# tomer196/GaUDI

Measured on AMD Instinct MI355X. Metric: guided molecules/sec (1000-step), higher is better.
Workload: dtype f32

## Files before the change

gaudi_amd/csrc/sampler_kernel.h:

```cpp
#pragma once
#include "edm_device.h"
#include "pred_device.h"
#include "w8_edm.h"
#include "w8_pred.h"

#ifndef GAUDI_STATIC_PRIO
#define GAUDI_STATIC_PRIO 0
#endif

namespace gaudi {

enum Mode { MODE_PHI = 0, MODE_SAMPLE = 1, MODE_PRED_FWD = 2, MODE_PRED_GRAD = 3, MODE_GUIDE = 4, MODE_NLL = 5 };

struct KParams {
  int mode, B, N, F, EW;
  int NR;
  int do_init, do_decode, guided;
  int s_hi, s_lo, T;
  const float* node_mask;
  const int* order;
  const uint32_t* edges;
  const float* emask;
  const int* npairs;
  const uint32_t* seginfo;
// ... 289 lines not shown
    base += align16((N + 1 + S + 1) / 2);
    for (int i = tid; i < N; i += kThreads) sSeg[i] = P.seginfo[b * N + i];
    for (int i = tid; i < N + 1; i += kThreads) sOff[i] = P.soff[(size_t)b * (N + 1) + i];
    for (int i = tid; i < S; i += kThreads) {
      sEdge[i] = P.edges[(size_t)b * S + i];
      sEm[i] = P.emask[(size_t)b * S + i];
      sIdx[i] = P.sidx[(size_t)b * S + i];
    }
    mg.N = N; mg.D = 3 + P.F; mg.S = S;
    mg.NC = P.ncols[b];
    mg.ntiles = P.npairs[b];
    mg.rounds = (mg.ntiles + w8::kWaves - 1) / w8::kWaves;
    mg.pubx = P.pubx;
    mg.pub_ch = P.pub_ch;
    mg.hk = P.hk_off;
    mg.side = P.side_off;
    mg.mask = sMask; mg.edge = sEdge; mg.em = sEm; mg.seg = sSeg; mg.soff = sOff; mg.sidx = sIdx;
    return base;
  }
  __device__ __forceinline__ static void set_rows(Graph& mg, const int* row, int ncomp, int NR) { mg.row = row; mg.ncomp = ncomp; mg.NR = NR; }
  __device__ __forceinline__ static Graph8Args gargs(const Graph& mg) {
    return Graph8Args{mg.N, mg.D, mg.S, mg.NC, mg.ntiles, mg.pubx, mg.pub_ch, mg.hk};
  }
  static constexpr bool kGlobalNodes = GN != 0 || PG;
  template <int HP>
  __device__ __forceinline__ static void edm(const EdmDev& W, const Graph& mg, float* net, const float* sZ, float* sEps,
                                             float* sMean, float t_val, int tid STAMP_DECL, float* gnode) {
#ifdef GAUDI_STAMPS
    w8::NetSmem<HP, SP, GN> sm;
    sm.carve(net, mg.N, mg.S, GN ? uni(gnode) : nullptr);
    sm.hk = w8::lds_at(mg.hk);
    w8::edm_forward<HP, SP, GN>(W, mg, sm, sZ, sEps, sMean, t_val, tid STAMP_ARGS);
#else
    (void)net; (void)sZ; (void)sEps; (void)sMean; (void)tid;
    edm8_call<HP, SP, GN, kFL>(W, gargs(mg), t_val, gnode);
#endif
  }
  template <int HP>
  __device__ __forceinline__ static void guide(const PredDev& W, const Graph& mg, float* net, float* sZ, float* sGrad, float* sTmp,
                                               float* sMean, float t_val, float sigma, const float* target_w, float scale,
                                               float* pred_out, float readout_div, float* stash, int tid STAMP_DECL, int phase,
                                               const float* dpred_ext, float* gnode, const float* dz_ext, const VtDev* vt,
                                               int b, int srow) {
#ifdef GAUDI_STAMPS
    (void)vt; (void)b; (void)srow;
    (void)dz_ext;
    w8::guidance_update<HP, SP, MR, GN, PG>(W, mg, net, sZ, sGrad, sTmp, sMean, t_val, sigma, target_w, scale, pred_out, readout_div, stash,
                                            mg.pubx, mg.pub_ch, tid STAMP_ARGS, phase, dpred_ext, (GN || PG) ? uni(gnode) : nullptr);
#else
    (void)sTmp;
    w8::PredSmem<HP, SP, GN, PG> sm;
    sm.carve(net, mg.N, mg.S, mg.pubx, gnode);
    if (phase != 2) pred_fwd8_call<HP, SP, MR, GN, kFL, PG, SD>(W, gargs(mg), t_val, stash, readout_div, gnode, SD != 0 ? mg.side : 0);
    if (vt != nullptr) vt_seed8(vt, b, srow, W.K, (int)(sm.pred - lds_base()));
    else w8::guidance_seed(W, sm, target_w, scale, pred_out, tid, phase, dpred_ext);
    if (phase == 1) return;
    pred_bwd8_call<HP, SP, MR, GN, kFL, PG>(W, gargs(mg), stash, readout_div, phase == 2 ? 1 : 0, gnode);
    if (dz_ext != nullptr) {
      for (int e = tid; e < mg.N * mg.D; e += kThreads) sGrad[e] += dz_ext[e];
      __syncthreads();
    }
    if (vt != nullptr) vt_norm8(vt, b, srow, W.K, mg.N * mg.D, (int)(sGrad - lds_base()));
    w8::guidance_apply(mg, sZ, sGrad, sMean, sigma, tid);
    if (vt != nullptr) vt_clip8(vt, b, srow, W.K, (int)(sMean - lds_base()));
#endif
  }
  template <int HP>
  __device__ __forceinline__ static void pred_entry(const PredDev& W, const Graph& mg, float* net, float* sZ, float* sGrad,
                                                    float* sTmp, float* sMean, float t_val, const float* dpred, bool want_grad,
                                                    float* pred_out, float readout_div, float* stash, int tid STAMP_DECL, float* gnode) {
    w8::predictor_entry<HP, SP, MR, GN, PG>(W, mg, net, sZ, sGrad, sTmp, sMean, t_val, dpred, want_grad, pred_out, readout_div, stash, mg.pubx,
                            mg.pub_ch, tid STAMP_ARGS, gnode);
  }
};
using V8 = V8T<0>;
using V8S = V8T<1>;
using V8H = V8T<2>;

__host__ __device__ inline int common_floats_base(int N, int D) { return 3 * align16(N * D) + align16(N) + 16; }

// ... 361 lines not shown
```

gaudi_amd/csrc/w8_edm.h:

```cpp
#pragma once
#include "edm_device.h"
#include "w8_common.h"
#include "w8_split.h"
#include "w8_nodes_f16.h"

namespace gaudi {
namespace w8 {

__host__ __device__ constexpr int gn_lds_buffers(int gn) { return gn == 2 ? 2 : 0; }
template <int HP, int SP = 0, int GN = 0>
struct NetSmem {
  static constexpr bool kGlobalNodes = GN != 0;
  float *h, *p, *q;
  float *agg, *agg1;
  float* ring;
  float *x, *x0;
  uint32_t *pmax, *qmax;
  float* hsc;
  f4* geo;
  float* d0;
  float* trans;
  float* vec;
  float* hk = nullptr;
  __host__ __device__ static int floats(int N, int S) {
// ... 115 lines not shown
    const float* ew = w + lay.emb_w();
    const float* eb = w + lay.emb_b();
    for (int idx = tid; idx < N * HP; idx += kThreads) {
      const int n = idx / HP, f = idx % HP;
      float acc = 0.f;
      const float m = mg.mask[n];
      for (int k = 0; k < F; ++k) acc += gload(ew + f * F1 + k) * (sZ[n * D + 3 + k] * m);
      acc += gload(ew + f * F1 + F) * t_val;
      sm.h[n * LD + f] = acc + gload(eb + f);
    }
  }
  __syncthreads();
  compute_geo(sm, mg, 0.f, tid, true);
  typename EdgeRing<HP, SP>::type ring;
  er_init<HP>(ring, sm.ring, W.ktail != 0, W.ws, W.hinv);
  static_assert(SP == 0 || NodeMath<SP>::kF16, "the split edge GEMMs take their column scales from the fp16 node GEMMs' row maxima");
  constexpr bool NH = NodeMath<SP>::kF16;
  constexpr bool RI = node_ring_idle(HP, SP, GN);
  constexpr bool STG = GN && !NH;
  float* const xs0 = sm.ring;
  float* const xs1 = sm.ring + stage_stride(N * LD);
  if constexpr (!RI) er_start<HP>(ring, wbe, lay.gcl(0, 0) + 2 * PK, wave, lane);
  typename NodePFSel<HP, NH>::type pf;
  node_prefetch_x<HP, NH, kAheadOne>(pf, wb, wbe, lay.gcl(0, 0), mg.NC, wave, lane, tw);
  auto hctx = [&]() {
    if constexpr (NH) {
      if constexpr (RI) return node_ctx_h<HP>(sm.ring, EdgeRing<HP, SP>::kFloats, mg.NC, W.hinv, tw, sm.hsc);
      else return node_ctx_h<HP>(ring.slot(ring.par ^ 1), EdgeRing<HP, SP>::kFloats / 2, mg.NC, W.hinv, tw, sm.hsc);
    } else {
      return NodeCtxH{1.f, nullptr, nullptr, tw, nullptr};
    }
  };
  const bool keep = NH && sm.hk != nullptr;
  bool h_kept = false;
  constexpr int NV = (7 * HP + 16 + kThreads - 1) / kThreads;
  VecPF<NV> vpf;
  vec_prefetch<NV, kThreads>(vpf, wb, lay.gcl(0, 0) + 6 * PK, 7 * HP + 16, tid);
  STAMP(ST_EDM_IO);

  for (int l = 0; l < W.L; ++l) {
    compute_geo(sm, mg, W.norm_constant, tid, false);
    STAMP(ST_GEO);
    for (int s = 0; s < W.S; ++s) {
      const int G = lay.gcl(l, s);
      const int Wnext_edge = s + 1 < W.S ? lay.gcl(l, s + 1) + 2 * PK : lay.equ(l) + 2 * PK;
      if constexpr (STG) stage_rows(xs0, sm.h, N * LD, wave, lane);
      for (int idx = tid; idx < N * (LD / 4); idx += kThreads) {
// ... 209 lines not shown
```

gaudi_amd/csrc/w8_nodes_f16.h:

```cpp
#pragma once
#include "w8_split.h"

namespace gaudi {
namespace w8 {


constexpr float kLoScale = 2048.f;
#ifndef GAUDI_NODE_ABLATE
#define GAUDI_NODE_ABLATE 0
#endif
constexpr int kAblateH = GAUDI_NODE_ABLATE;
#ifndef GAUDI_NODE_STAMPS
#define GAUDI_NODE_STAMPS 0
#endif
#ifndef GAUDI_NODE_PRIO
#define GAUDI_NODE_PRIO 1
#endif
struct NodeStampH {
  unsigned long long sum[8], last;
  __device__ __forceinline__ void start() { last = __builtin_amdgcn_s_memtime(); }
  __device__ __forceinline__ void mark(int i) {
    const unsigned long long t = __builtin_amdgcn_s_memtime();
    sum[i] += t - last;
    last = t;
// ... 103 lines not shown
}
template <int HP, class SRC>
__device__ __forceinline__ void split_rows_h(const SplitBufH& sb, const SRC& X_, int N, int wave, int lane) {
  const auto X = rows_of(X_);
  for (int n = wave; n < N; n += 2 * kWaves) {
    const int n2 = n + kWaves < N ? n + kWaves : n;
    SplitRowH a = split_row_load<HP>(X, n, lane), b = split_row_load<HP>(X, n2, lane);
    a.mx = wave_max_u32(a.mx);
    b.mx = wave_max_u32(b.mx);
    split_row_store<HP>(sb, a.x, a.mx, n, lane);
    if (n2 != n) split_row_store<HP>(sb, b.x, b.mx, n2, lane);
  }
}

__device__ __forceinline__ void lds_barrier() {
  asm volatile("s_waitcnt lgkmcnt(0)" ::: "memory");
  __builtin_amdgcn_s_barrier();
  asm volatile("" ::: "memory");
}

#ifndef GAUDI_NODE_DEPTH
#define GAUDI_NODE_DEPTH 3
#endif
#ifndef GAUDI_NODE_LATE
#define GAUDI_NODE_LATE 0
#endif
#ifndef GAUDI_NODE_TAIL_EARLY
#define GAUDI_NODE_TAIL_EARLY 0
#endif
template <int HP>
struct NodeGeoH {
  static constexpr int T = HP / 16;
  static constexpr int NTW = T > kWaves ? 2 : 1;
  static constexpr int nc = nh_chunks(HP);
  static constexpr int D = nc < GAUDI_NODE_DEPTH ? (nc > 0 ? nc : 1) : GAUDI_NODE_DEPTH;
  static constexpr bool odd = nh_odd(HP);
};
template <int NTW>
struct NodeSetH {
  u4 p[NTW][2];
};
template <int HP>
struct NodePFH {
  NodeSetH<NodeGeoH<HP>::NTW> s[NodeGeoH<HP>::D];
};

constexpr int kOOBBytes = (int)0x80000000u;
template <int HP>
struct TileLanesH {
  int vo[NodeGeoH<HP>::NTW];
  __device__ __forceinline__ TileLanesH(int wave, int lane, bool on = true) {
#pragma unroll
    for (int u = 0; u < NodeGeoH<HP>::NTW; ++u)
      vo[u] = (on && wave + kWaves * u < NodeGeoH<HP>::T) ? lane * 16 + (wave + kWaves * u) * 2048 : kOOBBytes;
  }
};
template <int HP, int NU = NodeGeoH<HP>::NTW>
__device__ __forceinline__ void nh_load(NodeSetH<NodeGeoH<HP>::NTW>& s, const WBuf& wh, int chunk_off, const TileLanesH<HP>& tl) {
#pragma unroll
  for (int u = 0; u < NU; ++u) {
    s.p[u][0] = __builtin_bit_cast(u4, __builtin_amdgcn_raw_buffer_load_b128(wh.r, tl.vo[u], chunk_off * 4, GAUDI_NODE_LOAD_AUX));
    s.p[u][1] = __builtin_bit_cast(u4, __builtin_amdgcn_raw_buffer_load_b128(wh.r, tl.vo[u] + 1024, chunk_off * 4, GAUDI_NODE_LOAD_AUX));
  }
}
constexpr int kAheadOne = 1, kAheadAll = 99;
template <int HP, int AHEAD = kAheadAll>
__device__ __forceinline__ void node_prefetch_h(NodePFH<HP>& pf, const WBuf& wh, int W , int wave, int lane) {
  constexpr int nd = AHEAD < NodeGeoH<HP>::D ? AHEAD : NodeGeoH<HP>::D;
  const TileLanesH<HP> tl(wave, lane);
  static_for<nd>([&](auto d_tag) {
    constexpr int d = decltype(d_tag)::value;
    nh_load<HP>(pf.s[d], wh, 2 * W + d * nh_chunk_floats(HP), tl);
  });
}

constexpr int kNodePlain = 0;
constexpr int kNodeFresh = 1;
constexpr int kNodeOneTile = 2;
constexpr int kTailRuntime = 0;
constexpr int kTailOne = 1;

struct NodeCtxH {
  float winv;
  float* split_a;
  float* split_b;
  bool ktail;
  float* scales;
  float* scales_b = nullptr;
};

struct YInitBias {};
struct YInitRows {
  const float* y;
};
template <int HP, int EPI, bool TWO, int MAXNT, int PIN = kAheadOne, int POUT = kAheadOne, int FL = kNodePlain, int TAIL = kTailRuntime,
          int NU = 0, class XB = const float*, class XA = const float*, class YI = YInitBias>
__device__ __forceinline__ void node_gemm_h(const WBuf& wh, int Wa, const XA& sXa, bool do_split_a, int Wb, const XB& sXb,
                                            const float* sBias, float* sY, const float* sRes, const float* sMask, int N, int wave,
                                            int lane, const NodeCtxH& cx, NodePFH<HP>& pf, int nextW = -1, float* gPre = nullptr,
                                            uint32_t* sMaxOut = nullptr ,
                                            NodeStampH* ns = nullptr, const YI& yinit = YI{}) {
  (void)ns;
  (void)yinit;
  using G = NodeGeoH<HP>;
  constexpr int T = G::T, LD = HP + 4, NTW = NU > 0 ? NU : G::NTW, nc = G::nc, D = G::D;
  constexpr int kIn = PIN < D ? PIN : D, kOut = POUT < D ? POUT : D;
  constexpr int kLate = nc < D ? 0 : (GAUDI_NODE_LATE < kOut ? GAUDI_NODE_LATE : kOut);
  constexpr int TQ = TAIL == kTailOne ? 1 : 4;
  const bool ktail = TAIL == kTailOne ? true : cx.ktail;
  constexpr bool kFresh = FL == kNodeFresh;
  const int c = lane & 15, g = lane >> 4;
  const int nt = (MAXNT < 2 || N <= 16) ? 1 : (MAXNT < 3 || N <= 32) ? 2 : 3;
  const bool seq = TWO && cx.split_b == cx.split_a;
  const SplitBufH sa{cx.split_a, nt, cx.scales}, sb{cx.split_b, nt, cx.scales_b != nullptr ? cx.scales_b : cx.scales + kScaleFloatsH};
  const int bpos = nh_bpos(c, g);
  const TileLanesH<HP> tl(wave, lane);
  const TileLanesH<HP> tl_next(wave, lane, nextW >= 0);
  const int Wn = nextW >= 0 ? nextW : Wa;
  static_for<D>([&](auto d_tag) {
    constexpr int d = decltype(d_tag)::value;
    if constexpr (d >= kIn) nh_load<HP, NTW>(pf.s[d], wh, 2 * Wa + d * nh_chunk_floats(HP), tl);
  });
  float ta[NTW][TQ], tb[NTW][TQ];
  if constexpr (G::odd) {
#pragma unroll
    for (int u = 0; u < NTW; ++u) {
      const int t = wave + kWaves * u < T ? wave + kWaves * u : 0;
#pragma unroll
      for (int q = 0; q < TQ; ++q) {
        const int ln = ((q == 0 || !ktail) && wave + kWaves * u < T) ? lane : kOOBLane;
// ... 40 lines not shown
#pragma unroll
    for (int u = 0; u < NTW; ++u) acc1[j][u] = mfma_h(s.p[u][0], b.l, acc1[j][u]);
#pragma unroll
    for (int u = 0; u < NTW; ++u) acc0[j][u] = mfma_h(s.p[u][0], b.h, acc0[j][u]);
#pragma unroll
    for (int u = 0; u < NTW; ++u) acc1[j][u] = mfma_h(s.p[u][1], b.h, acc1[j][u]);
  };
  auto tail_steps = [&](const SplitBufH& s_, const float (&tw)[NTW][TQ], auto j_tag) {
    constexpr int j = decltype(j_tag)::value;
    if constexpr (G::odd) {
      const float* xt = s_.tail(HP) + j * 256 + g * 16 + c;
#pragma unroll
      for (int u = 0; u < NTW; ++u) y[j][u] = mfma1(tw[u][0], xt[0], y[j][u]);
      if constexpr (TQ > 1) {
        if (!ktail) {
#pragma unroll
          for (int q = 1; q < TQ; ++q)
#pragma unroll
            for (int u = 0; u < NTW; ++u) y[j][u] = mfma1(tw[u][q], xt[64 * q], y[j][u]);
        }
      }
    }
  };
  constexpr bool kTailEarly = GAUDI_NODE_TAIL_EARLY != 0;
  auto tail_early = [&](const SplitBufH& s_, const float (&tw)[NTW][TQ]) {
    if constexpr (kTailEarly && G::odd)
      static_for<MAXNT>([&](auto j_tag) {
        if (decltype(j_tag)::value < nt) tail_steps(s_, tw, j_tag);
      });
  };
  auto fold = [&](const SplitBufH& s_, const float (&tw)[NTW][TQ]) {
    static_for<MAXNT>([&](auto j_tag) {
      constexpr int j = decltype(j_tag)::value;
      if (j < nt) {
        if constexpr (!kTailEarly) tail_steps(s_, tw, j_tag);
        const float sc = s_.scale(HP)[j * 16 + c] * cx.winv;
#pragma unroll
        for (int u = 0; u < NTW; ++u) {
          y[j][u] = y[j][u] + (acc0[j][u] + acc1[j][u] * (1.0f / kLoScale)) * sc;
          acc0[j][u] = splat(0.f);
          acc1[j][u] = splat(0.f);
        }
      }
    });
  };
  auto source = [&](auto src_tag, const SplitBufH& s_) {
    constexpr int src = decltype(src_tag)::value;
    constexpr bool last_src = !TWO || src == 1;
    const int Wcur = src == 0 ? Wa : Wb;
    BH bcur = bld(s_, 0, 0);
    static_for<nc>([&](auto i_tag) {
      constexpr int i = decltype(i_tag)::value;
      constexpr int d = i % D;
      BH bnext = bcur;
      if constexpr (i + 1 < nc) bnext = bld(s_, i + 1, 0);
      __builtin_amdgcn_sched_barrier(0);
      mm(pf.s[d], bcur, 0);
      if constexpr (MAXNT >= 2) {
        if (nt >= 2) {
          mm(pf.s[d], bld(s_, i, 1), 1);
          if constexpr (MAXNT >= 3) {
            if (nt >= 3) mm(pf.s[d], bld(s_, i, 2), 2);
          }
        }
      }
      __builtin_amdgcn_sched_barrier(0);
      if (!(kAblateH & 4)) {
        if constexpr (i + D < nc) nh_load<HP, NTW>(pf.s[d], wh, 2 * Wcur + (i + D) * nh_chunk_floats(HP), tl);
        else if constexpr (!last_src) nh_load<HP, NTW>(pf.s[d], wh, 2 * Wb + d * nh_chunk_floats(HP), tl);
        else if constexpr (d < kOut - kLate) nh_load<HP, NTW>(pf.s[d], wh, 2 * Wn + d * nh_chunk_floats(HP), tl_next);
      }
      __builtin_amdgcn_sched_barrier(0);
      bcur = bnext;
    });
  };
  auto late = [&](auto d_tag) {
    constexpr int d = decltype(d_tag)::value;
    if constexpr (d >= kOut - kLate && d < kOut) {
      __builtin_amdgcn_sched_barrier(0);
      if (!(kAblateH & 4)) nh_load<HP, NTW>(pf.s[d], wh, 2 * Wn + d * nh_chunk_floats(HP), tl_next);
      __builtin_amdgcn_sched_barrier(0);
    }
  };
  NSTAMP(3);
#if GAUDI_NODE_PRIO
  if constexpr (!kFresh)
    if ((GAUDI_NODE_PRIO == 1 && wave >= kWaves / 2) || (GAUDI_NODE_PRIO == 2 && wave < kWaves / 2)) __builtin_amdgcn_s_setprio(1);
#endif
  tail_early(sa, ta);
  source(std::integral_constant<int, 0>{}, sa);
  NSTAMP(4);
  if constexpr (!TWO) late(std::integral_constant<int, kOut - kLate>{});
  fold(sa, ta);
  NSTAMP(5);
  if constexpr (TWO) {
    if (seq) {
      lds_barrier();
      split_rows_h<HP>(sb, sXb, N, wave, kFresh ? fresh(lane) : lane);
      lds_barrier();
    }
    tail_early(sb, tb);
    source(std::integral_constant<int, 1>{}, sb);
    late(std::integral_constant<int, kOut - kLate>{});
    fold(sb, tb);
  }
  static_for<D>([&](auto d_tag) {
    if constexpr (decltype(d_tag)::value > kOut - kLate) late(d_tag);
  });
#if GAUDI_NODE_PRIO
  if constexpr (!kFresh) __builtin_amdgcn_s_setprio(0);
#endif
  const int le = kFresh ? fresh(lane) : lane, ce = le & 15, ge = le >> 4;
  static_for<MAXNT>([&](auto j_tag) {
    constexpr int j = decltype(j_tag)::value;
    if (j < nt) {
#pragma unroll
      for (int u = 0; u < NTW; ++u) {
        const int t = wave + kWaves * u;
        const int nd = j * 16 + ce;
        f4 yy = y[j][u];
        if (t < T && nd < N) {
          float* dst = sY + nd * LD + 16 * t + 4 * ge;
          const bool pad = G::odd && ktail && t == T - 1 && ge > 0;
          if (pad) yy = splat(0.f);
          if (gPre != nullptr) nstash_store((f4*)(gPre + nd * HP + 16 * t + 4 * ge), yy);
          if (sMaxOut != nullptr) atomicMax(sMaxOut + nd, umax(umax(absbits(yy[0]), absbits(yy[1])), umax(absbits(yy[2]), absbits(yy[3]))));
          if (!pad) {
            if (EPI == EPI_SILU) yy = silu4v(yy);
            if (EPI == EPI_RESIDUAL_MASK) {
              const f4 r = *(const f4*)(sRes + nd * LD + 16 * t + 4 * ge);
              yy = (r + yy) * sMask[nd];
// ... 108 lines not shown
    side_compute<HP, s>(job, a, lane);
    __builtin_amdgcn_sched_barrier(0);
    side_issue<HP, s + 1>(job, a, lane);
    __builtin_amdgcn_sched_barrier(0);
    ring.par ^= 1;
  });
}

#ifndef GAUDI_NODE_F16
#define GAUDI_NODE_F16 1
#endif
template <int SP>
struct NodeMath {
  static constexpr bool kF16 = SP != 0 && GAUDI_NODE_F16 != 0;
};
template <int HP, bool NH>
struct NodePFSel {
  using type = NodePF<HP>;
};
template <int HP>
struct NodePFSel<HP, true> {
  using type = NodePFH<HP>;
};
template <int HP, bool NH, int AHEAD, class PF>
__device__ __forceinline__ void node_prefetch_x(PF& pf, const WBuf& wb, const WBuf& wbe, int W, int N, int wave, int lane, bool tw) {
  if constexpr (NH) node_prefetch_h<HP, AHEAD>(pf, wbe, W, wave, lane);
  else node_prefetch<HP>(pf, wb, W, wave, lane, tw);
}
template <int HP, int EPI, bool TWO, int GN, bool NH, int PIN, int POUT, int FL = kNodePlain, int XBS = 0, class PF>
__device__ __forceinline__ void node_gemm_x(const WBuf& wb, const WBuf& wbe, int Wa, const float* Xa, const float* XaS, bool split_a, int Wb,
                                            const float* Xb, const float* XbS, const float* sBias, float* sY, const float* sRes,
                                            const float* sMask, int N, int wave, int lane, bool tw, const NodeCtxH& cx, PF& pf,
                                            int nextW = -1, float* gPre = nullptr, uint32_t* sMaxOut = nullptr,
                                            const float* Xb1 = nullptr, float xb_div = 1.f) {
  static_assert(XBS == 0 || (NH && GN == 0 && TWO), "summed second sources: the fp16-pair form of the resident kernels");
  if constexpr (NH) {
    constexpr int MAXNT = GN ? 3 : FL == kNodeOneTile ? 1 : 2;
    constexpr int TAIL = FL == kNodeOneTile && nh_odd(HP) ? kTailOne : kTailRuntime;
    if constexpr (XBS == 0)
      node_gemm_h<HP, EPI, TWO, MAXNT, PIN, POUT, FL, TAIL>(wbe, Wa, Xa, split_a, Wb, Xb, sBias, sY, sRes, sMask, N, wave, lane, cx, pf, nextW,
                                                            gPre, sMaxOut);
    else
      node_gemm_h<HP, EPI, TWO, MAXNT, PIN, POUT, FL, TAIL>(wbe, Wa, Xa, split_a, Wb, RowsSum<XBS == 2>{Xb, Xb1, xb_div}, sBias, sY, sRes, sMask, N,
                                                            wave, lane, cx, pf, nextW, gPre, sMaxOut);
  } else if constexpr (GN != 0) {
    node_gemm_n<HP, EPI, true, 3>(wb, Wa, XaS, Wb, XbS, sBias, sY, sRes, sMask, N, wave, lane, tw, &pf, nextW, gPre);
  } else {
    node_gemm<HP, EPI, true>(wb, Wa, Xa, Wb, Xb, sBias, sY, sRes, sMask, N, wave, lane, tw, &pf, nextW, gPre);
  }
}
__host__ __device__ constexpr bool node_ring_idle(int HP, int SP, bool GN) {
  return GN || (SP != 0 && GAUDI_NODE_F16 != 0 && (SP == 2 || HP < 48));
}
template <int HP>
__device__ __forceinline__ NodeCtxH node_ctx_h(float* region, int cap, int N, float winv, bool ktail, float* scales) {
  const int nct = N <= 16 ? 1 : N <= 32 ? 2 : 3;
  const int need = nh_split_floats(HP, nct);
  return NodeCtxH{winv, region, 2 * need <= cap ? region + need : region, ktail, scales};
}
__host__ __device__ constexpr int nh_keep_floats(int HP, int N) { return nh_split_floats(HP, N <= 16 ? 1 : N <= 32 ? 2 : 3) + kScaleFloatsH; }
template <int HP>
__device__ __forceinline__ NodeCtxH node_ctx_keep(const NodeCtxH& cx, float* keep, int N) {
  const int nct = N <= 16 ? 1 : N <= 32 ? 2 : 3;
  return NodeCtxH{cx.winv, keep + kScaleFloatsH, cx.split_a, cx.ktail, keep, cx.scales};
  (void)nct;
}

// ... 3 lines not shown
```

gaudi_amd/csrc/w8_pred.h:

```cpp
#pragma once
#include "pred_device.h"
#include "w8_edm.h"

namespace gaudi {
namespace w8 {

template <int HP, int SP = 0, int GN = 0, bool PG = false>
struct PredSmem {
  static_assert(!(PG && GN != 0), "PG is a variant of the resident kernels");
  static_assert(!GN || SP != 0, "global node buffers: split edge GEMMs only (the fp32 form's publish buffer starts in b0 / b1)");
  static constexpr bool kGlobalNodes = GN != 0;
  float *b2, *b3, *b4;
  float *b0, *b1;
  float* ring;
  float* pub;
  float *x, *x0, *dx;
  uint32_t *pmax, *qmax;
  float* hsc;
  f4* geo;
  float *d0, *trans, *dd0;
  float* pred;
  float* vec;
  float* hk = nullptr;
  float* side = nullptr;
// ... 66 lines not shown
  {
    const float* ew = w + lay.emb_w();
    const float* eb = w + lay.emb_b();
    for (int idx = tid; idx < N * HP; idx += kThreads) {
      const int n = idx / HP, f = idx % HP;
      float acc = 0.f;
      const float m = mg.mask[n];
      for (int k = 0; k < F; ++k) acc += gload(ew + f * F1 + k) * (sZ[n * D + 3 + k] * m);
      acc += gload(ew + f * F1 + F) * t_val;
      h[n * LD + f] = acc + gload(eb + f);
    }
  }
  __syncthreads();
  compute_geo(sm, mg, 0.f, tid, true);
  typename EdgeRing<HP, SP>::type ring;
  er_init<HP>(ring, sm.ring, W.ktail != 0, W.ws, W.hinv);
  constexpr bool NH = NodeMath<SP>::kF16;
  constexpr bool RI = node_ring_idle(HP, SP, GN);
  constexpr bool STG = GN && !NH;
  float* const xs0 = sm.ring;
  float* const xs1 = sm.ring + stage_stride(N * LD);
  if constexpr (!RI) er_start<HP>(ring, wbe, lay.layer(0) + 2 * HP * HP, wave, lane);
  typename NodePFSel<HP, NH>::type pf;
  node_prefetch_x<HP, NH, kAheadOne>(pf, wb, wbe, lay.layer(0), mg.NC, wave, lane, tw);
  auto hctx = [&]() {
    if constexpr (NH) {
      if constexpr (RI) return node_ctx_h<HP>(sm.ring, EdgeRing<HP, SP>::kFloats, mg.NC, W.hinv, tw, sm.hsc);
      else return node_ctx_h<HP>(ring.slot(ring.par ^ 1), EdgeRing<HP, SP>::kFloats / 2, mg.NC, W.hinv, tw, sm.hsc);
    } else {
      return NodeCtxH{1.f, nullptr, nullptr, tw, nullptr};
    }
  };
  const bool keep = NH && sm.hk != nullptr;
  constexpr bool kSideA = (SD & 1) != 0;
  static_assert(!kSideA || (NH && !MR && GN == 0 && !RI && FL == kNodeOneTile), "the side job is a form of the resident N1 kernel");
  constexpr int NV = (PredLayerW::vec_count(HP) + kThreads - 1) / kThreads;
  VecPF<NV> vpf;
  vec_prefetch<NV, kThreads>(vpf, wb, PredLayerW::vec_off(lay.layer(0), HP), PredLayerW::vec_count(HP), tid);

  for (int l = 0; l < W.L; ++l) {
    const bool last = l == W.L - 1;
    const PredLayerW Lw(w, lay.layer(l), HP, sm.vec);
    const bool side_l = kSideA && sm.side != nullptr && !last && (tw || !SplitGeo<HP, SP == 0 ? 1 : SP>::kTailOK);
    vec_commit<NV, kThreads>(vpf, sm.vec, PredLayerW::vec_count(HP), tid);
    if constexpr (STG) stage_rows(xs0, h, N * LD, wave, lane);
    for (int idx = tid; idx < N * LD; idx += kThreads) {
      agg[idx] = 0.f;
      agg1[idx] = 0.f;
    }
    if (tid < N) {
      sm.pmax[tid] = 0u;
      sm.qmax[tid] = 0u;
    }
    float* st = stash + (size_t)l * (3 * N * HP + 4 * N);
    for (int idx = tid; idx < N; idx += kThreads) gstore4((f4*)(st + 3 * N * HP) + idx, *(const f4*)(sm.x + 4 * idx));
    compute_geo(sm, mg, 1.0f, tid, false);
    if constexpr (STG) stage_wait();
    else __syncthreads();
// ... 86 lines not shown
      }
      if constexpr (MR) {
        if (++rd < mg.rounds) goto pred_fwd_round;
      }
    }
    __syncthreads();
    STAMP(ST_BARRIER);
    constexpr bool SUM = NH && GN == 0;
    if constexpr (!SUM) {
      if constexpr (STG) stage_rows(xs0, h, N * LD, wave, lane);
      for (int idx = tid; idx < N * (HP / 4); idx += kThreads) {
        const int n = idx / (HP / 4), f = 4 * (idx % (HP / 4));
        if constexpr (STG)
          *(f4*)(xs1 + n * LD + f) = *(const f4*)(agg + n * LD + f) + *(const f4*)(agg1 + n * LD + f);
        else
          *(f4*)(agg + n * LD + f) = *(const f4*)(agg + n * LD + f) + *(const f4*)(agg1 + n * LD + f);
      }
      if constexpr (STG) stage_wait();
      else __syncthreads();
    }
    STAMP(ST_MISC);
    if constexpr (kSideA) {
      if (side_l)
        node_gemm_h<HP, EPI_SILU, false, 1, kAheadOne, kAheadOne, FL, nh_odd(HP) ? kTailOne : kTailRuntime>(
            wbe, Lw.Wn1a, RowsSum<false>{agg, agg1, 1.f}, true, -1, (const float*)nullptr, nullptr, p, nullptr, nullptr, mg.NC, wave, lane,
            hctx(), pf, Lw.Wn2, st + 2 * N * HP , nullptr, nullptr, YInitRows{sm.side});
    }
    if (!side_l)
    node_gemm_x<HP, EPI_SILU, true, GN, NH, kAheadOne, kAheadOne, FL, SUM ? 1 : 0>(
        wb, wbe, Lw.Wn1h, h, xs0, !keep, Lw.Wn1a, agg, xs1, Lw.bn1, p, nullptr, nullptr, mg.NC, wave, lane, tw,
        keep ? node_ctx_keep<HP>(hctx(), sm.hk, mg.NC) : hctx(), pf, Lw.Wn2, st + 2 * N * HP , nullptr, agg1);
    STAMP(ST_NODE);
    __syncthreads();
    STAMP(ST_BARRIER);
    vec_prefetch<NV, kThreads>(vpf, wb, PredLayerW::vec_off(lay.layer(l + 1 < W.L ? l + 1 : l), HP), PredLayerW::vec_count(HP), tid);
    if constexpr (STG) {
      stage_rows(xs0, p, N * LD, wave, lane);
      stage_wait();
    }
    node_gemm_x<HP, EPI_RESIDUAL_MASK, false, GN, NH, kAheadOne, kAheadOne, FL>(wb, wbe, Lw.Wn2, p, xs0, true, -1, nullptr, nullptr, Lw.bn2, h, h, mg.mask, mg.NC, wave,
                                                     lane, tw, hctx(), pf, l + 1 < W.L ? lay.layer(l + 1) : -1);
    if (!last) coord_update(sm, mg, 1.0f, tid);
    STAMP(ST_NODE);
    __syncthreads();
    STAMP(ST_BARRIER);
  }
  {
// ... 54 lines not shown
    for (int idx = tid; idx < N * HP; idx += kThreads) {
      const int n = idx / HP, f = idx % HP;
      float acc = 0.f;
      for (int k = 0; k < K; ++k) acc += (dpred[k] / readout_div) * gload(ow + k * HP + f);
      dh[n * LD + f] = acc * mg.mask[n];
    }
    for (int idx = tid; idx < N * 4; idx += kThreads) sm.dx[idx] = 0.f;
    for (int idx = tid; idx < S; idx += kThreads) sm.dd0[idx] = 0.f;
  }
  __syncthreads();

  typename EdgeRing<HP, SP>::type ring;
  er_init<HP>(ring, sm.ring, W.ktail != 0, W.ws, W.hinv);
  constexpr bool NH = NodeMath<SP>::kF16;
  constexpr bool RI = node_ring_idle(HP, SP, GN);
  constexpr bool STG = GN && !NH;
  float* const xs0 = sm.ring;
  float* const xs1 = sm.ring + stage_stride(N * LD);
  if constexpr (!RI) {
    const int L0 = lay.layer(W.L - 1);
    er_start<HP>(ring, wbe, L0 + 9 * HP * HP , wave, lane);
  }
  typename NodePFSel<HP, NH>::type pf;
  node_prefetch_x<HP, NH, kAheadOne>(pf, wb, wbe, lay.layer(W.L - 1) + 13 * HP * HP , mg.NC, wave, lane, tw);
  auto hctx = [&]() {
    if constexpr (NH) {
      if constexpr (RI) return node_ctx_h<HP>(sm.ring, EdgeRing<HP, SP>::kFloats, mg.NC, W.hinv, tw, sm.hsc);
      else return node_ctx_h<HP>(ring.slot(ring.par ^ 1), EdgeRing<HP, SP>::kFloats / 2, mg.NC, W.hinv, tw, sm.hsc);
    } else {
      return NodeCtxH{1.f, nullptr, nullptr, tw, nullptr};
    }
  };
  constexpr int NV = (PredLayerW::vec_count(HP) + kThreads - 1) / kThreads;
  VecPF<NV> vpf;
  vec_prefetch<NV, kThreads>(vpf, wb, PredLayerW::vec_off(lay.layer(W.L - 1), HP), PredLayerW::vec_count(HP), tid);
  STAMP(ST_X1);
  for (int l = W.L - 1; l >= 0; --l) {
    const bool last = l == W.L - 1;
    const PredLayerW Lw(w, lay.layer(l), HP, sm.vec);
    const float* st = stash + (size_t)l * (3 * N * HP + 4 * N);
    {
      const int tid = fresh(tid_);
      const int n4 = N * (HP / 4);
#ifdef GAUDI_DIAG_HOT_STASH
      const f4* sp = (const f4*)W.w;
      const f4* sq = (const f4*)(W.w + N * HP);
      const f4* sn = (const f4*)(W.w + 2 * N * HP);
// ... 186 lines not shown
              if (t >= t0 && t < t1) *(f4*)(row + 16 * t) = du[t];
          }
        }
        __syncthreads();
        STAMP(ST_B_V);
        const int nf4 = (t1 - t0) * 4;
        for (int idx = tid; idx < N * nf4; idx += kThreads) {
          const int n = idx / nf4, f = 4 * (idx % nf4);
          const uint32_t sg = mg.seg[n];
          const int rs = sg >> 16, rl = sg & 0xffff;
          f4 sp = splat(0.f), sq = splat(0.f);
          for (int k = 0; k < rl; ++k) sp += *(const f4*)(pub + (rs + k) * PLD + f);
          const int s0 = mg.soff[n], s1 = mg.soff[n + 1];
          for (int k = s0; k < s1; ++k) sq += *(const f4*)(pub + (int)mg.sidx[k] * PLD + f);
          *(f4*)(B2 + n * LD + 16 * t0 + f) = sp;
          *(f4*)(B4 + n * LD + 16 * t0 + f) = sq;
        }
        STAMP(ST_B_EV);
        __syncthreads();
        STAMP(ST_B_CP);
      }
      if (SP != 0 && !RI && l > 0)
        er_start<HP>(ring, wbe, lay.layer(l - 1) + 10 * HP * HP , wave, lane);
      node_prefetch_x<HP, NH, kAheadOne>(pf, wb, wbe, Lw.At, mg.NC, wave, lane, tw);
      STAMP(ST_BWD_COL);
    }
    for (int idx = tid; idx < N * 3; idx += kThreads) {
      const int n = idx / 3, d = idx % 3;
      const uint32_t sg = mg.seg[n];
      const int rs = sg >> 16, rl = sg & 0xffff;
      float acc = sm.dx[4 * n + d];
      for (int k = 0; k < rl; ++k) acc += sm.trans[4 * (rs + k) + d];
      const int s0 = mg.soff[n], s1 = mg.soff[n + 1];
      for (int k = s0; k < s1; ++k) acc -= sm.trans[4 * (int)mg.sidx[k] + d];
      sm.dx[4 * n + d] = acc;
    }
    vec_prefetch<NV, kThreads>(vpf, wb, PredLayerW::vec_off(lay.layer(l > 0 ? l - 1 : 0), HP), PredLayerW::vec_count(HP), tid);
    if constexpr (STG) {
      stage_rows(xs0, B2, N * LD, wave, lane);
      stage_rows(xs1, B4, N * LD, wave, lane);
      stage_wait();
    }
    node_gemm_x<HP, EPI_ACCUM, true, GN, NH, kAheadOne, kAheadOne, FL>(wb, wbe, Lw.At, B2, xs0, true, Lw.Bmt, B4, xs1, nullptr, dh, dh, nullptr, mg.NC, wave, lane, tw,
                                             hctx(), pf, l > 0 ? lay.layer(l - 1) + 13 * HP * HP : -1);
    __syncthreads();
    STAMP(ST_BWD_NODE);
  }
// ... 119 lines not shown
```

gaudi_amd/flops.py:

```python
from __future__ import annotations


def _edm_as_written(N, H, F, L, S):
    E, Nn = N * N, N
    gcl = 2 * E * ((2 * H + 2) * H + H * H + H) + 2 * Nn * 3 * H * H
    equ = 2 * E * ((2 * H + 2) * H + H * H + H)
    return L * (S * gcl + equ) + 4 * Nn * (F + 1) * H


def _pred_as_written(N, H, F, L, K):
    E, Nn = N * N, N
    lay = 2 * E * ((2 * H + 2) * H + H * H + H) + 2 * E * (H * H + H) + 2 * Nn * 3 * H * H
    return L * lay + 2 * Nn * ((F + 1) * H + H * K)


def step_flops_as_written(N, F, edm, pred=None, K=5):
    f = _edm_as_written(N, edm["nf"], F, edm["n_layers"], edm.get("inv_sublayers", 1))
    if pred is not None:
        f += 2 * _pred_as_written(N, pred["nf"], F, pred["n_layers"], K)
    return f


def step_flops_useful(n_live_edges, n_nodes, F, edm, pred=None, K=5):
    E, Nn = n_live_edges, n_nodes
# ... 24 lines not shown
FLOP_MFMA_F32 = 2048
FLOP_MFMA_BF16 = 16384
PEAK_F32_TFLOPS = 157.3
PEAK_BF16_TFLOPS = 2516.6


def _has_ktail(nf, HP):
    return nf % 16 == 4 and HP - nf == 12


def step_mfma_counts(edge_units, ncols, edm, pred=None, variant="w4", max_col_tiles=2):
    ncols = int(ncols)
    nt = 1 if ncols <= 16 else (3 if max_col_tiles >= 3 and 32 < ncols <= 48 else 2 * (((ncols + 15) // 16 + 1) // 2))
    if variant == "w4":
        waves, pairs = 4, int(sum(int(v) for v in edge_units))
        tiles16 = 2 * pairs
    else:
        waves, tiles16 = 8, int(edge_units)

    def node(T, kt, nf):
        if variant == "w4":
            return kt * 4 * (-(-T // waves)) * waves * nt, 0
        if variant == "w8s":
            slots = waves * (2 if T > waves else 1)
            mats = kt // T
            tail = (1 if _has_ktail(nf, 16 * T) else 4) if T % 2 else 0
            return mats * slots * tail * nt, mats * (T // 2) * 3 * slots * nt
        tail44 = _has_ktail(nf, 16 * T) and 16 * T in (208, 48)
        return kt * 4 * (T - 0.75 if tail44 else T) * nt, 0

    def edge(T, nf):
        tail = variant != "w4" and _has_ktail(nf, 16 * T)
        if variant == "w8s":
            tail = tail and T % 2 == 1 and T >= 3
            nc = (T + 1) // 2 - (1 if tail else 0)
            return (T if tail else 0), nc * T * 3
        return T * (4 * T - 3 if tail else 4 * T), 0

    f32 = bf = 0
    Te = _pad_hidden_kernel(edm["nf"]) // 16
    L, S = edm["n_layers"], edm.get("inv_sublayers", 1)
    e32, ebf = edge(Te, edm["nf"])
    n32, n16 = node(Te, (5 * S + 2) * Te, edm["nf"])
    f32 += L * (n32 + (S + 1) * tiles16 * e32)
    bf += L * (n16 + (S + 1) * tiles16 * ebf)
    if pred is not None:
        Tp = _pad_hidden_kernel(pred["nf"]) // 16
        Lp = pred["n_layers"]
        e32, ebf = edge(Tp, pred["nf"])
        n_edge = 2 * (2 * Lp - 1)
        n32, n16 = node(Tp, 5 * Tp, pred["nf"])
        f32 += 2 * Lp * n32 + n_edge * tiles16 * e32
        bf += 2 * Lp * n16 + n_edge * tiles16 * ebf
    return f32, bf


def step_mfma_issued(edge_units, ncols, edm, pred=None, variant="w4", max_col_tiles=2):
    return step_mfma_counts(edge_units, ncols, edm, pred, variant, max_col_tiles)[0]


def step_weight_stream_bytes(edm, pred=None, variant="w8s", rounds=1):
    def node_b(T):
        return (16 * T) ** 2 * 4
# ... 21 lines not shown
```

Baseline: 224.3.

## Specialize node GEMMs per wave by slot count to skip idle slots

When output tiles split unevenly across the eight waves, each wave now picks at runtime a kernel instantiation compiled for its own slot count (one or two tiles). Waves with one tile no longer issue MFMAs or weight prefetches for an empty second slot. Unused late-prefetch and early-tail experiment knobs are removed. The cost is extra template instantiations, which grows code size and may add instruction-cache pressure and wave divergence at sync points.

Result: faster. 229.4 (median of 6 runs) (+2.3%).

```diff
diff --git a/gaudi_amd/csrc/sampler_kernel.h b/gaudi_amd/csrc/sampler_kernel.h
--- a/gaudi_amd/csrc/sampler_kernel.h
+++ b/gaudi_amd/csrc/sampler_kernel.h
@@ -335,6 +335,7 @@
   __device__ __forceinline__ static Graph8Args gargs(const Graph& mg) {
     return Graph8Args{mg.N, mg.D, mg.S, mg.NC, mg.ntiles, mg.pubx, mg.pub_ch, mg.hk};
   }
+  __device__ __forceinline__ static int slot_wave() { return __builtin_amdgcn_readfirstlane((int)(threadIdx.x >> 6)); }
   static constexpr bool kGlobalNodes = GN != 0 || PG;
   template <int HP>
   __device__ __forceinline__ static void edm(const EdmDev& W, const Graph& mg, float* net, const float* sZ, float* sEps,
@@ -346,7 +347,12 @@
     w8::edm_forward<HP, SP, GN>(W, mg, sm, sZ, sEps, sMean, t_val, tid STAMP_ARGS);
 #else
     (void)net; (void)sZ; (void)sEps; (void)sMean; (void)tid;
-    edm8_call<HP, SP, GN, kFL>(W, gargs(mg), t_val, gnode);
+    if constexpr (N1 && w8::node_uneven_slots<HP>()) {
+      if (slot_wave() + w8::kWaves < HP / 16) edm8_call<HP, SP, GN, kFL + w8::kNodeSlots2>(W, gargs(mg), t_val, gnode);
+      else edm8_call<HP, SP, GN, kFL + w8::kNodeSlots1>(W, gargs(mg), t_val, gnode);
+    } else {
+      edm8_call<HP, SP, GN, kFL>(W, gargs(mg), t_val, gnode);
+    }
 #endif
   }
   template <int HP>
@@ -364,11 +370,25 @@
     (void)sTmp;
     w8::PredSmem<HP, SP, GN, PG> sm;
     sm.carve(net, mg.N, mg.S, mg.pubx, gnode);
-    if (phase != 2) pred_fwd8_call<HP, SP, MR, GN, kFL, PG, SD>(W, gargs(mg), t_val, stash, readout_div, gnode, SD != 0 ? mg.side : 0);
+    constexpr bool kClasses = N1 && w8::node_uneven_slots<HP>();
+    const bool two_slots = kClasses && slot_wave() + w8::kWaves < HP / 16;
+    if (phase != 2) {
+      if constexpr (kClasses) {
+        if (two_slots) pred_fwd8_call<HP, SP, MR, GN, kFL + w8::kNodeSlots2, PG, SD>(W, gargs(mg), t_val, stash, readout_div, gnode, SD != 0 ? mg.side : 0);
+        else pred_fwd8_call<HP, SP, MR, GN, kFL + w8::kNodeSlots1, PG, SD>(W, gargs(mg), t_val, stash, readout_div, gnode, SD != 0 ? mg.side : 0);
+      } else {
+        pred_fwd8_call<HP, SP, MR, GN, kFL, PG, SD>(W, gargs(mg), t_val, stash, readout_div, gnode, SD != 0 ? mg.side : 0);
+      }
+    }
     if (vt != nullptr) vt_seed8(vt, b, srow, W.K, (int)(sm.pred - lds_base()));
     else w8::guidance_seed(W, sm, target_w, scale, pred_out, tid, phase, dpred_ext);
     if (phase == 1) return;
-    pred_bwd8_call<HP, SP, MR, GN, kFL, PG>(W, gargs(mg), stash, readout_div, phase == 2 ? 1 : 0, gnode);
+    if constexpr (kClasses) {
+      if (two_slots) pred_bwd8_call<HP, SP, MR, GN, kFL + w8::kNodeSlots2, PG>(W, gargs(mg), stash, readout_div, phase == 2 ? 1 : 0, gnode);
+      else pred_bwd8_call<HP, SP, MR, GN, kFL + w8::kNodeSlots1, PG>(W, gargs(mg), stash, readout_div, phase == 2 ? 1 : 0, gnode);
+    } else {
+      pred_bwd8_call<HP, SP, MR, GN, kFL, PG>(W, gargs(mg), stash, readout_div, phase == 2 ? 1 : 0, gnode);
+    }
     if (dz_ext != nullptr) {
       for (int e = tid; e < mg.N * mg.D; e += kThreads) sGrad[e] += dz_ext[e];
       __syncthreads();
diff --git a/gaudi_amd/csrc/w8_edm.h b/gaudi_amd/csrc/w8_edm.h
--- a/gaudi_amd/csrc/w8_edm.h
+++ b/gaudi_amd/csrc/w8_edm.h
@@ -161,7 +161,7 @@
   float* const xs1 = sm.ring + stage_stride(N * LD);
   if constexpr (!RI) er_start<HP>(ring, wbe, lay.gcl(0, 0) + 2 * PK, wave, lane);
   typename NodePFSel<HP, NH>::type pf;
-  node_prefetch_x<HP, NH, kAheadOne>(pf, wb, wbe, lay.gcl(0, 0), mg.NC, wave, lane, tw);
+  node_prefetch_x<HP, NH, kAheadOne, FL>(pf, wb, wbe, lay.gcl(0, 0), mg.NC, wave, lane, tw);
   auto hctx = [&]() {
     if constexpr (NH) {
       if constexpr (RI) return node_ctx_h<HP>(sm.ring, EdgeRing<HP, SP>::kFloats, mg.NC, W.hinv, tw, sm.hsc);
diff --git a/gaudi_amd/csrc/w8_nodes_f16.h b/gaudi_amd/csrc/w8_nodes_f16.h
--- a/gaudi_amd/csrc/w8_nodes_f16.h
+++ b/gaudi_amd/csrc/w8_nodes_f16.h
@@ -149,12 +149,6 @@
 #ifndef GAUDI_NODE_DEPTH
 #define GAUDI_NODE_DEPTH 3
 #endif
-#ifndef GAUDI_NODE_LATE
-#define GAUDI_NODE_LATE 0
-#endif
-#ifndef GAUDI_NODE_TAIL_EARLY
-#define GAUDI_NODE_TAIL_EARLY 0
-#endif
 template <int HP>
 struct NodeGeoH {
   static constexpr int T = HP / 16;
@@ -191,19 +185,25 @@
   }
 }
 constexpr int kAheadOne = 1, kAheadAll = 99;
-template <int HP, int AHEAD = kAheadAll>
+template <int HP, int AHEAD = kAheadAll, int NU = 0>
 __device__ __forceinline__ void node_prefetch_h(NodePFH<HP>& pf, const WBuf& wh, int W , int wave, int lane) {
   constexpr int nd = AHEAD < NodeGeoH<HP>::D ? AHEAD : NodeGeoH<HP>::D;
   const TileLanesH<HP> tl(wave, lane);
   static_for<nd>([&](auto d_tag) {
     constexpr int d = decltype(d_tag)::value;
-    nh_load<HP>(pf.s[d], wh, 2 * W + d * nh_chunk_floats(HP), tl);
+    nh_load<HP, (NU > 0 ? NU : NodeGeoH<HP>::NTW)>(pf.s[d], wh, 2 * W + d * nh_chunk_floats(HP), tl);
   });
 }
 
 constexpr int kNodePlain = 0;
 constexpr int kNodeFresh = 1;
 constexpr int kNodeOneTile = 2;
+constexpr int kNodeSlots1 = 4, kNodeSlots2 = 8;
+__host__ __device__ constexpr bool node_one_tile(int FL) { return (FL & 3) == kNodeOneTile; }
+template <int HP>
+__host__ __device__ constexpr bool node_uneven_slots() { return NodeGeoH<HP>::NTW == 2 && NodeGeoH<HP>::T < 2 * kWaves; }
+template <int HP>
+__host__ __device__ constexpr int node_slots(int FL) { return node_one_tile(FL) && node_uneven_slots<HP>() ? FL >> 2 : 0; }
 constexpr int kTailRuntime = 0;
 constexpr int kTailOne = 1;
 
@@ -232,7 +232,6 @@
   using G = NodeGeoH<HP>;
   constexpr int T = G::T, LD = HP + 4, NTW = NU > 0 ? NU : G::NTW, nc = G::nc, D = G::D;
   constexpr int kIn = PIN < D ? PIN : D, kOut = POUT < D ? POUT : D;
-  constexpr int kLate = nc < D ? 0 : (GAUDI_NODE_LATE < kOut ? GAUDI_NODE_LATE : kOut);
   constexpr int TQ = TAIL == kTailOne ? 1 : 4;
   const bool ktail = TAIL == kTailOne ? true : cx.ktail;
   constexpr bool kFresh = FL == kNodeFresh;
@@ -319,18 +318,11 @@
       }
     }
   };
-  constexpr bool kTailEarly = GAUDI_NODE_TAIL_EARLY != 0;
-  auto tail_early = [&](const SplitBufH& s_, const float (&tw)[NTW][TQ]) {
-    if constexpr (kTailEarly && G::odd)
-      static_for<MAXNT>([&](auto j_tag) {
-        if (decltype(j_tag)::value < nt) tail_steps(s_, tw, j_tag);
-      });
-  };
   auto fold = [&](const SplitBufH& s_, const float (&tw)[NTW][TQ]) {
     static_for<MAXNT>([&](auto j_tag) {
       constexpr int j = decltype(j_tag)::value;
       if (j < nt) {
-        if constexpr (!kTailEarly) tail_steps(s_, tw, j_tag);
+        tail_steps(s_, tw, j_tag);
         const float sc = s_.scale(HP)[j * 16 + c] * cx.winv;
 #pragma unroll
         for (int u = 0; u < NTW; ++u) {
@@ -365,29 +357,19 @@
       if (!(kAblateH & 4)) {
         if constexpr (i + D < nc) nh_load<HP, NTW>(pf.s[d], wh, 2 * Wcur + (i + D) * nh_chunk_floats(HP), tl);
         else if constexpr (!last_src) nh_load<HP, NTW>(pf.s[d], wh, 2 * Wb + d * nh_chunk_floats(HP), tl);
-        else if constexpr (d < kOut - kLate) nh_load<HP, NTW>(pf.s[d], wh, 2 * Wn + d * nh_chunk_floats(HP), tl_next);
+        else if constexpr (d < kOut) nh_load<HP, NTW>(pf.s[d], wh, 2 * Wn + d * nh_chunk_floats(HP), tl_next);
       }
       __builtin_amdgcn_sched_barrier(0);
       bcur = bnext;
     });
   };
-  auto late = [&](auto d_tag) {
-    constexpr int d = decltype(d_tag)::value;
-    if constexpr (d >= kOut - kLate && d < kOut) {
-      __builtin_amdgcn_sched_barrier(0);
-      if (!(kAblateH & 4)) nh_load<HP, NTW>(pf.s[d], wh, 2 * Wn + d * nh_chunk_floats(HP), tl_next);
-      __builtin_amdgcn_sched_barrier(0);
-    }
-  };
   NSTAMP(3);
 #if GAUDI_NODE_PRIO
   if constexpr (!kFresh)
     if ((GAUDI_NODE_PRIO == 1 && wave >= kWaves / 2) || (GAUDI_NODE_PRIO == 2 && wave < kWaves / 2)) __builtin_amdgcn_s_setprio(1);
 #endif
-  tail_early(sa, ta);
   source(std::integral_constant<int, 0>{}, sa);
   NSTAMP(4);
-  if constexpr (!TWO) late(std::integral_constant<int, kOut - kLate>{});
   fold(sa, ta);
   NSTAMP(5);
   if constexpr (TWO) {
@@ -396,14 +378,9 @@
       split_rows_h<HP>(sb, sXb, N, wave, kFresh ? fresh(lane) : lane);
       lds_barrier();
     }
-    tail_early(sb, tb);
     source(std::integral_constant<int, 1>{}, sb);
-    late(std::integral_constant<int, kOut - kLate>{});
     fold(sb, tb);
   }
-  static_for<D>([&](auto d_tag) {
-    if constexpr (decltype(d_tag)::value > kOut - kLate) late(d_tag);
-  });
 #if GAUDI_NODE_PRIO
   if constexpr (!kFresh) __builtin_amdgcn_s_setprio(0);
 #endif
@@ -558,9 +535,9 @@
 struct NodePFSel<HP, true> {
   using type = NodePFH<HP>;
 };
-template <int HP, bool NH, int AHEAD, class PF>
+template <int HP, bool NH, int AHEAD, int FL = kNodePlain, class PF>
 __device__ __forceinline__ void node_prefetch_x(PF& pf, const WBuf& wb, const WBuf& wbe, int W, int N, int wave, int lane, bool tw) {
-  if constexpr (NH) node_prefetch_h<HP, AHEAD>(pf, wbe, W, wave, lane);
+  if constexpr (NH) node_prefetch_h<HP, AHEAD, node_slots<HP>(FL)>(pf, wbe, W, wave, lane);
   else node_prefetch<HP>(pf, wb, W, wave, lane, tw);
 }
 template <int HP, int EPI, bool TWO, int GN, bool NH, int PIN, int POUT, int FL = kNodePlain, int XBS = 0, class PF>
@@ -571,14 +548,15 @@
                                             const float* Xb1 = nullptr, float xb_div = 1.f) {
   static_assert(XBS == 0 || (NH && GN == 0 && TWO), "summed second sources: the fp16-pair form of the resident kernels");
   if constexpr (NH) {
-    constexpr int MAXNT = GN ? 3 : FL == kNodeOneTile ? 1 : 2;
-    constexpr int TAIL = FL == kNodeOneTile && nh_odd(HP) ? kTailOne : kTailRuntime;
+    constexpr int MAXNT = GN ? 3 : node_one_tile(FL) ? 1 : 2;
+    constexpr int TAIL = node_one_tile(FL) && nh_odd(HP) ? kTailOne : kTailRuntime;
+    constexpr int NU = node_slots<HP>(FL);
     if constexpr (XBS == 0)
-      node_gemm_h<HP, EPI, TWO, MAXNT, PIN, POUT, FL, TAIL>(wbe, Wa, Xa, split_a, Wb, Xb, sBias, sY, sRes, sMask, N, wave, lane, cx, pf, nextW,
-                                                            gPre, sMaxOut);
+      node_gemm_h<HP, EPI, TWO, MAXNT, PIN, POUT, FL, TAIL, NU>(wbe, Wa, Xa, split_a, Wb, Xb, sBias, sY, sRes, sMask, N, wave, lane, cx, pf, nextW,
+                                                                gPre, sMaxOut);
     else
-      node_gemm_h<HP, EPI, TWO, MAXNT, PIN, POUT, FL, TAIL>(wbe, Wa, Xa, split_a, Wb, RowsSum<XBS == 2>{Xb, Xb1, xb_div}, sBias, sY, sRes, sMask, N,
-                                                            wave, lane, cx, pf, nextW, gPre, sMaxOut);
+      node_gemm_h<HP, EPI, TWO, MAXNT, PIN, POUT, FL, TAIL, NU>(wbe, Wa, Xa, split_a, Wb, RowsSum<XBS == 2>{Xb, Xb1, xb_div}, sBias, sY, sRes, sMask,
+                                                                N, wave, lane, cx, pf, nextW, gPre, sMaxOut);
   } else if constexpr (GN != 0) {
     node_gemm_n<HP, EPI, true, 3>(wb, Wa, XaS, Wb, XbS, sBias, sY, sRes, sMask, N, wave, lane, tw, &pf, nextW, gPre);
   } else {
diff --git a/gaudi_amd/csrc/w8_pred.h b/gaudi_amd/csrc/w8_pred.h
--- a/gaudi_amd/csrc/w8_pred.h
+++ b/gaudi_amd/csrc/w8_pred.h
@@ -112,7 +112,7 @@
   float* const xs1 = sm.ring + stage_stride(N * LD);
   if constexpr (!RI) er_start<HP>(ring, wbe, lay.layer(0) + 2 * HP * HP, wave, lane);
   typename NodePFSel<HP, NH>::type pf;
-  node_prefetch_x<HP, NH, kAheadOne>(pf, wb, wbe, lay.layer(0), mg.NC, wave, lane, tw);
+  node_prefetch_x<HP, NH, kAheadOne, FL>(pf, wb, wbe, lay.layer(0), mg.NC, wave, lane, tw);
   auto hctx = [&]() {
     if constexpr (NH) {
       if constexpr (RI) return node_ctx_h<HP>(sm.ring, EdgeRing<HP, SP>::kFloats, mg.NC, W.hinv, tw, sm.hsc);
@@ -123,7 +123,7 @@
   };
   const bool keep = NH && sm.hk != nullptr;
   constexpr bool kSideA = (SD & 1) != 0;
-  static_assert(!kSideA || (NH && !MR && GN == 0 && !RI && FL == kNodeOneTile), "the side job is a form of the resident N1 kernel");
+  static_assert(!kSideA || (NH && !MR && GN == 0 && !RI && node_one_tile(FL)), "the side job is a form of the resident N1 kernel");
   constexpr int NV = (PredLayerW::vec_count(HP) + kThreads - 1) / kThreads;
   VecPF<NV> vpf;
   vec_prefetch<NV, kThreads>(vpf, wb, PredLayerW::vec_off(lay.layer(0), HP), PredLayerW::vec_count(HP), tid);
@@ -256,7 +256,7 @@
     STAMP(ST_MISC);
     if constexpr (kSideA) {
       if (side_l)
-        node_gemm_h<HP, EPI_SILU, false, 1, kAheadOne, kAheadOne, FL, nh_odd(HP) ? kTailOne : kTailRuntime>(
+        node_gemm_h<HP, EPI_SILU, false, 1, kAheadOne, kAheadOne, FL, nh_odd(HP) ? kTailOne : kTailRuntime, node_slots<HP>(FL)>(
             wbe, Lw.Wn1a, RowsSum<false>{agg, agg1, 1.f}, true, -1, (const float*)nullptr, nullptr, p, nullptr, nullptr, mg.NC, wave, lane,
             hctx(), pf, Lw.Wn2, st + 2 * N * HP , nullptr, nullptr, YInitRows{sm.side});
     }
@@ -357,7 +357,7 @@
     er_start<HP>(ring, wbe, L0 + 9 * HP * HP , wave, lane);
   }
   typename NodePFSel<HP, NH>::type pf;
-  node_prefetch_x<HP, NH, kAheadOne>(pf, wb, wbe, lay.layer(W.L - 1) + 13 * HP * HP , mg.NC, wave, lane, tw);
+  node_prefetch_x<HP, NH, kAheadOne, FL>(pf, wb, wbe, lay.layer(W.L - 1) + 13 * HP * HP , mg.NC, wave, lane, tw);
   auto hctx = [&]() {
     if constexpr (NH) {
       if constexpr (RI) return node_ctx_h<HP>(sm.ring, EdgeRing<HP, SP>::kFloats, mg.NC, W.hinv, tw, sm.hsc);
@@ -590,7 +590,7 @@
       }
       if (SP != 0 && !RI && l > 0)
         er_start<HP>(ring, wbe, lay.layer(l - 1) + 10 * HP * HP , wave, lane);
-      node_prefetch_x<HP, NH, kAheadOne>(pf, wb, wbe, Lw.At, mg.NC, wave, lane, tw);
+      node_prefetch_x<HP, NH, kAheadOne, FL>(pf, wb, wbe, Lw.At, mg.NC, wave, lane, tw);
       STAMP(ST_BWD_COL);
     }
     for (int idx = tid; idx < N * 3; idx += kThreads) {
diff --git a/gaudi_amd/flops.py b/gaudi_amd/flops.py
--- a/gaudi_amd/flops.py
+++ b/gaudi_amd/flops.py
@@ -70,7 +70,7 @@
         if variant == "w4":
             return kt * 4 * (-(-T // waves)) * waves * nt, 0
         if variant == "w8s":
-            slots = waves * (2 if T > waves else 1)
+            slots = T if lean else waves * (2 if T > waves else 1)
             mats = kt // T
             tail = (1 if _has_ktail(nf, 16 * T) else 4) if T % 2 else 0
             return mats * slots * tail * nt, mats * (T // 2) * 3 * slots * nt
@@ -87,6 +87,8 @@
 
     f32 = bf = 0
     Te = _pad_hidden_kernel(edm["nf"]) // 16
+    lean = (variant == "w8s" and ncols <= 16 and max_col_tiles < 3 and 16 * Te == 192 and
+            (pred is None or (_pad_hidden_kernel(pred["nf"]) == 208 and _has_ktail(pred["nf"], 208))))
     L, S = edm["n_layers"], edm.get("inv_sublayers", 1)
     e32, ebf = edge(Te, edm["nf"])
     n32, n16 = node(Te, (5 * S + 2) * Te, edm["nf"])
```
